# spvkgn/vorbis-aotuv-lancer

Hardware: AMD Instinct MI355X
Metric: realtime-stream-equivalents/node (44.1kHz stereo q5) + MDCT HBM GB/s (higher is better)
Workload: dtype f32

## Files before the change

vorbis_aotuv_lancer_amd/csrc/capi_encoder.cpp:

```cpp
#include <hip/hip_runtime.h>
#include <stdlib.h>
#include <string.h>
#include <functional>
#include <string>
#include <algorithm>
#include <thread>
#include <vector>

#include "vorbis_mi355x.h"
#include "setup_host.h"
#include "batch.h"
#include "kernels.h"
#include "mdct_kernel.h"
#include "vbm_internal.h"

extern "C" int vbm_launch_spread_flags(const vbm_batch *b, hipStream_t st);
vbm_setup_host *vbm_setup_handle_host(vbm_setup_handle *h);

static const int kMaxWS = 8;

struct vbm_encoder {
    vbm_setup_host *H;
    const vbm_setup *hs;
    int S, ch, cap;
// ... 447 lines not shown
    b.mix_makes_qf = vbm_mix_can_make_qf(&b);
    {
        const vbm_map &m = s->map[b.W];
        const vbm_psy &p = s->psy[block_mode];
        unsigned seen = 0;
        b.couple_parallel = 1;
        for (int i = 0; i < m.coupling_steps; i++) {
            unsigned bits = (1u << m.coupling_mag[i]) | (1u << m.coupling_ang[i]);
            if (seen & bits) b.couple_parallel = 0;
            seen |= bits;
        }
        const int partition = p.normal_p ? p.normal_partition : 16;
        int lowpassr = s->block_lowpassr[b.W ? 1 : 0];
        if (lowpassr % p.normal_partition) lowpassr = (lowpassr / p.normal_partition + 1) * p.normal_partition;
        b.couple_parts = (lowpassr + partition - 1) / partition;
        int m6end = p.tonefix_end < lowpassr ? p.tonefix_end : lowpassr;
        b.couple_m6parts = m.coupling_steps ? (m6end + partition - 1) / partition : 0;
        if (b.couple_parts > b.n / 8 + 1) b.couple_parallel = 0;
        b.couple_fast = 0;
        if (partition == 32 && p.normal_partition == 32 && (b.n % 32) == 0) {
            if (m.coupling_steps == 0) b.couple_fast = 1;
            else if (m.coupling_steps == 1 && e->ch == 2 && b.couple_parallel) b.couple_fast = 2;
        }
        b.pack_submaps = m.submaps;
        for (int i = 0; i < m.submaps && i < 16; i++) {
            const vbm_residue &r = s->residue[m.residuesubmap[i]];
            b.pack_partvals[i] = (r.end - r.begin) / r.grouping;
            b.pack_spp[i] = r.grouping;
        }
    }
}

static vbm_batch slice_of(const vbm_batch &f, int sb0, int nsb)
{
    vbm_batch v = f;
    const size_t cb0 = (size_t)sb0 * f.ch;
    const size_t ct = cb0 >> 6, stl = (size_t)sb0 >> 6;
    v.nsb = nsb;
    v.ncb = nsb * f.ch;
    v.stream_id += sb0; v.wflags += sb0;
    v.pcm += cb0 * f.N; v.mdct_bm += cb0 * f.n; v.logfft_bm += cb0 * f.n; v.qf_bm += cb0 * f.n;
    v.local_ampmax += cb0; v.wflags_cb += cb0; v.poste += cb0; v.post_valid += cb0; v.nonzero += cb0;
    v.post_valid_blob += cb0; v.nonzero_blob += cb0;
    v.global_ampmax += sb0; v.packet_bytes += sb0; v.packet_bits += sb0; v.packet_bits_blob += sb0;
    if (v.packet_bytes_blob) { v.packet_bytes_blob += sb0; v.choice += sb0; v.packetT_blob += stl * 64 * (size_t)f.max_packet_bytes; }
    const size_t co = ct * f.slab_words;
    v.mdctT += co; v.logmdctT += co; v.noiseT += co; v.toneT += co; v.logmaskT += co;
    v.epeakT += co; v.npeakT += co;
    v.postT += co; v.postT_blob += co; v.floor_outT += co; v.iworkT += co;
    v.floor_outT_blob += co; v.iworkT_blob += co;
    const size_t so = stl * f.sb_slab_words;
    v.partwordT += so; v.workvqT += so; v.m6defT += so; v.vqlenT += so; v.vqoffT += so;
    v.partwordT_blob += so; v.m6defT_blob += so; v.vqlenT_blob += so; v.vqoffT_blob += so;
    v.vqcodeT += stl * f.vq_slab_words; v.vqcodeT_blob += stl * f.vq_slab_words;
    v.packetT += stl * 64 * (size_t)f.max_packet_bytes;
    return v;
}

static int managed_front(const vbm_batch &v, hipStream_t q)
{
    static const int sel[3] = {1, 2, 0}, slot[3] = {VBM_PACKETBLOBS / 2, VBM_PACKETBLOBS - 1, 0};
    for (int t = 0; t < 3; t++) {
        vbm_batch f = v;
        f.postT = v.postT_blob + (size_t)slot[t] * (VBM_VIF_POSIT + 2) * 64;
        f.post_valid = v.post_valid_blob + (size_t)slot[t] * v.L;
        if (vbm_launch_mix_managed(&f, sel[t], q) || vbm_launch_floor_fit(&f, q)) return -2;
    }
    if (vbm_launch_block_state_managed(&v, q) || vbm_launch_floor_interp(&v, q)) return -2;
    return 0;
}

static int managed_back(const vbm_batch &v, uint8_t *d_packets, hipStream_t q, const std::function<int()> &before_choose = nullptr)
{
    vbm_batch f = v;
    f.nblobs = VBM_PACKETBLOBS;
    vbm_blob_select(f, 0);
    if (vbm_launch_floor_encode(&f, q)) return -2;
    if (f.couple_fast) {
        if (vbm_launch_couple_quantize(&f, q)) return -2;
    } else {
        for (int k = 0; k < VBM_PACKETBLOBS; k++) {
            vbm_batch g = v;
            vbm_blob_select(g, k);
            if (vbm_launch_couple_quantize(&g, q)) return -2;
        }
    }
    if (vbm_launch_pack(&f, q)) return -2;
    if (before_choose && before_choose()) return -2;
    return vbm_launch_bitrate_choose(&v, d_packets, q);
}


static int launch_transforms(vbm_encoder *e, const vbm_batch &v, hipStream_t q, bool timed)
{
    const vbm_setup *d = vbm_setup_device_ptrs(e->H);
    const int W = v.W, short_n = e->hs->blocksizes[0];
    const uint8_t *wf = W ? v.wflags_cb : nullptr;
    RUN(vbm_launch_spread_flags(&v, q));
    {
        stage_scope t(e, timed, 0, q);
        RUN(vbm_launch_window_mdct(v.pcm, v.mdct_bm, wf, d->mdct_trig[W], d->window[W], d->window[0], v.N, short_n, 1, v.ncb,
                                   0, v.d_nsb, e->ch, q));
    }
    stage_scope t(e, timed, 1, q);
    RUN(vbm_launch_window_fft_log(v.pcm, v.logfft_bm, v.local_ampmax, wf, d->fft_wa[W], d->window[W], d->window[0], v.N,
                                  short_n, v.ncb, v.d_nsb, e->ch, q));
    return VBM_OK;
}

static int launch_psy(vbm_encoder *e, const vbm_batch &v, hipStream_t q, bool timed, int side = -1)
{
    const int lines = e->hs->psy[v.block_mode].total_octave_lines;
    hipError_t err;
    { stage_scope t(e, timed, 3, q); RUN(vbm_launch_prologue(&v, q)); }
    if (side >= 0) {
        hipStream_t qa = e->aux[side];
        if ((err = hipEventRecord(e->ev_aux_fork[side], q)) != hipSuccess) return vbm_set_hip_error(err, "hipEventRecord");
        if ((err = hipStreamWaitEvent(qa, e->ev_aux_fork[side], 0)) != hipSuccess) return vbm_set_hip_error(err, "hipStreamWaitEvent");
        { stage_scope t(e, timed, 5, qa); RUN(vbm_launch_tonemask(&v, lines, qa)); }
        if ((err = hipEventRecord(e->ev_aux_join[side], qa)) != hipSuccess) return vbm_set_hip_error(err, "hipEventRecord");
        { stage_scope t(e, timed, 4, q); RUN(vbm_launch_noisemask(&v, q)); }
        if ((err = hipStreamWaitEvent(q, e->ev_aux_join[side], 0)) != hipSuccess) return vbm_set_hip_error(err, "hipStreamWaitEvent");
    } else {
        { stage_scope t(e, timed, 4, q); RUN(vbm_launch_noisemask(&v, q)); }
        { stage_scope t(e, timed, 5, q); RUN(vbm_launch_tonemask(&v, lines, q)); }
    }
    stage_scope t(e, timed, 6, q);
    if (e->hs->managed) RUN(managed_front(v, q));
    else { RUN(vbm_launch_mix(&v, q)); RUN(vbm_launch_block_state(&v, q)); }
    return VBM_OK;
}

static int launch_back(vbm_encoder *e, const vbm_batch &v, hipStream_t q, bool timed, uint8_t *d_packets,
                       const std::function<int()> &before_choose = nullptr)
{
    if (e->hs->managed) {
        stage_scope t(e, timed, 10, q);
        RUN(managed_back(v, d_packets, q, before_choose));
        return VBM_OK;
    }
    { stage_scope t(e, timed, 7, q); RUN(vbm_launch_floor_fit(&v, q)); }
    { stage_scope t(e, timed, 8, q); RUN(vbm_launch_floor_encode(&v, q)); }
    { stage_scope t(e, timed, 9, q); RUN(vbm_launch_couple_quantize(&v, q)); }
    stage_scope t(e, timed, 10, q);
    RUN(vbm_launch_pack(&v, q));
    return VBM_OK;
}

static int copy_packets(vbm_encoder *e, const vbm_batch &v, uint8_t *d_packets, int *d_packet_bytes, int sb0, hipStream_t q,
                        bool timed)
{
    stage_scope t(e, timed, 11, q);
    if (d_packets && !e->hs->managed)
        RUN(vbm_launch_untranspose_i32((const int *)v.packetT, (int *)(d_packets + (size_t)sb0 * e->max_packet_bytes),
                                       e->max_packet_bytes / 4, (size_t)(e->max_packet_bytes / 4) * 64, v.nsb, q));
    if (d_packet_bytes) {
        hipError_t err = hipMemcpyAsync(d_packet_bytes + sb0, v.packet_bytes, v.nsb * sizeof(int), hipMemcpyDeviceToDevice, q);
        if (err != hipSuccess) return vbm_set_hip_error(err, "hipMemcpyAsync(packet_bytes)");
    }
    return VBM_OK;
}

extern "C" int vbm_analysis_batch(vbm_encoder *e, int block_mode, int nsb, const int *stream_ids,
                                  const uint8_t *wflags, const float *d_pcm, uint8_t *d_packets,
                                  int *d_packet_bytes, void *stream)
{
    return vbm_analysis_batch2(e, block_mode, nsb, stream_ids, wflags, d_pcm, d_packets, d_packet_bytes, stream, stream);
}

extern "C" int vbm_analysis_batch2(vbm_encoder *e, int block_mode, int nsb, const int *stream_ids,
                                   const uint8_t *wflags, const float *d_pcm, uint8_t *d_packets,
                                   int *d_packet_bytes, void *stream_front, void *stream_back)
{
    void *stream = stream_front;
    if (!e || block_mode < 0 || block_mode > 3 || nsb < 0 || nsb > e->cap) return VBM_EINVAL;
    if (nsb == 0) return VBM_OK;
    if (!stream_ids || !wflags || !d_pcm) return VBM_EINVAL;
    if (((uintptr_t)d_pcm & 15) || ((uintptr_t)d_packets & 3)) return VBM_EINVAL;
    const vbm_setup *s = e->hs;
    if (s->modes < 2 && (block_mode >> 1)) return VBM_EINVAL;
    for (int i = 0; i < nsb; i++)
        if (stream_ids[i] < 0 || stream_ids[i] >= e->S) return VBM_EINVAL;
    hipStream_t st = (hipStream_t)stream;
    hipStream_t sback = (hipStream_t)stream_back;
    const bool two = (sback != st);
    hipError_t err;
    {
        int rcj = vbm_analysis_round_join(e, stream);
        if (rcj) return rcj;
        for (int ww = 0; ww < e->nws; ww++)
            for (int m = 0; m < 4; m++)
                if (e->reuse_pending[ww][m]) {
                    if ((err = hipStreamWaitEvent((hipStream_t)stream, e->ev_done[ww][m], 0)) != hipSuccess)
                        return vbm_set_hip_error(err, "hipStreamWaitEvent");
                    e->reuse_pending[ww][m] = false;
                }
        e->round_w = -1;
    }
    const int w = e->next;
    e->next = (e->next + 1) % e->nws;
    e->cur = w;
    if (e->back_pending[w]) {
        if ((err = hipStreamWaitEvent(st, e->ev_back[w], 0)) != hipSuccess) return vbm_set_hip_error(err, "hipStreamWaitEvent");
        e->back_pending[w] = false;
    }
    if ((int)e->last_ids[w].size() != nsb || memcmp(e->last_ids[w].data(), stream_ids, nsb * sizeof(int)) ||
        memcmp(e->last_flags[w].data(), wflags, nsb)) {
        e->seen.assign(e->S, 0);
        for (int i = 0; i < nsb; i++) {
            if (e->seen[stream_ids[i]]) { g_vbm_err = "a stream id appears twice in one batch"; return VBM_EINVAL; }
            e->seen[stream_ids[i]] = 1;
        }
        const int t = e->stage_turn;
        e->stage_turn ^= 1;
        (void)hipEventSynchronize(e->ev_stage[t]);
        memcpy(e->h_ids[t], stream_ids, nsb * sizeof(int));
        memcpy(e->h_flags[t], wflags, nsb);
        if ((err = hipMemcpyAsync(e->d_stream_id[w], e->h_ids[t], nsb * sizeof(int), hipMemcpyHostToDevice, st)) != hipSuccess)
            return vbm_set_hip_error(err, "hipMemcpyAsync(stream_ids)");
        if ((err = hipMemcpyAsync(e->d_wflags[w], e->h_flags[t], nsb, hipMemcpyHostToDevice, st)) != hipSuccess)
            return vbm_set_hip_error(err, "hipMemcpyAsync(wflags)");
        (void)hipEventRecord(e->ev_stage[t], st);
        e->last_ids[w].assign(stream_ids, stream_ids + nsb);
        e->last_flags[w].assign(wflags, wflags + nsb);
    }

    vbm_batch b;
    configure(e, b, block_mode, nsb, d_pcm, w);
    e->last_nsb = nsb;
    e->last_mode = block_mode;

    const int tiles = (nsb + 63) / 64;
    int nsplit = e->nsplit < tiles ? e->nsplit : tiles;
    if (nsplit < 1) nsplit = 1;
    const int nback = nsplit;
    if (two) nsplit = 1;

    int rc;
    const size_t ev_need = (size_t)2 * (kFront + (size_t)(nsplit > nback ? nsplit : nback) * kBack);
    const bool prof = e->profiling && e->prof_calls < e->prof_max_calls && e->events_used + ev_need <= e->events.size();
    vbm_debug_delay_point(VBM_DP_BATCH_FRONT, st);
    if ((rc = launch_transforms(e, b, st, prof))) return rc;
    if (two) {
        if ((rc = launch_psy(e, b, st, prof, e->overlap_branches ? 0 : -1))) return rc;
        if ((err = hipEventRecord(e->ev_front[w], st)) != hipSuccess) return vbm_set_hip_error(err, "hipEventRecord");
        for (int part = 0; part < nback; part++) {
            const int t0 = (int)((long)tiles * part / nback), t1 = (int)((long)tiles * (part + 1) / nback);
            const int sb0 = t0 * 64, sb1 = (t1 * 64 < nsb) ? t1 * 64 : nsb;
            if (sb1 <= sb0) continue;
            hipStream_t qb = part ? e->sub[part] : sback;
            if ((err = hipStreamWaitEvent(qb, e->ev_front[w], 0)) != hipSuccess) return vbm_set_hip_error(err, "hipStreamWaitEvent");
            vbm_debug_delay_point(VBM_DP_BATCH_BACK, qb);
            vbm_batch vs = nback > 1 ? slice_of(b, sb0, sb1 - sb0) : b;
            if ((rc = launch_back(e, vs, qb, prof, d_packets ? d_packets + (size_t)sb0 * e->max_packet_bytes : nullptr)) ||
                (rc = copy_packets(e, vs, d_packets, d_packet_bytes, sb0, qb, prof)))
                return rc;
            if (part) {
                if ((err = hipEventRecord(e->ev_join[part], qb)) != hipSuccess) return vbm_set_hip_error(err, "hipEventRecord");
                if ((err = hipStreamWaitEvent(sback, e->ev_join[part], 0)) != hipSuccess) return vbm_set_hip_error(err, "hipStreamWaitEvent");
            }
        }
        if ((err = hipEventRecord(e->ev_back[w], sback)) != hipSuccess) return vbm_set_hip_error(err, "hipEventRecord");
        e->back_pending[w] = true;
    } else {
        if (nsplit > 1 && (err = hipEventRecord(e->ev_fork, st)) != hipSuccess) return vbm_set_hip_error(err, "hipEventRecord");
        for (int part = 0; part < nsplit; part++) {
            const int t0 = (int)((long)tiles * part / nsplit), t1 = (int)((long)tiles * (part + 1) / nsplit);
            const int sb0 = t0 * 64, sb1 = (t1 * 64 < nsb) ? t1 * 64 : nsb;
            if (sb1 <= sb0) continue;
            hipStream_t q = st;
            vbm_batch v = b;
            if (nsplit > 1) {
                q = e->sub[part];
                v = slice_of(b, sb0, sb1 - sb0);
                if ((err = hipStreamWaitEvent(q, e->ev_fork, 0)) != hipSuccess) return vbm_set_hip_error(err, "hipStreamWaitEvent");
            }
            if ((rc = launch_psy(e, v, q, prof, e->overlap_branches ? part : -1)) ||
                (rc = launch_back(e, v, q, prof, d_packets ? d_packets + (size_t)sb0 * e->max_packet_bytes : nullptr)) ||
                (rc = copy_packets(e, v, d_packets, d_packet_bytes, sb0, q, prof)))
                return rc;
            if (nsplit > 1) {
                if ((err = hipEventRecord(e->ev_join[part], q)) != hipSuccess) return vbm_set_hip_error(err, "hipEventRecord");
                if ((err = hipStreamWaitEvent(st, e->ev_join[part], 0)) != hipSuccess) return vbm_set_hip_error(err, "hipStreamWaitEvent");
            }
        }
    }
    if (prof) { e->prof_calls++; e->prof_blocks += nsb; }
    return VBM_OK;
}

struct type_job {
    int m, w;
    int lane0, bound;
    const int *d_nsb;
    const float *pcm;
    uint8_t *d_packets;
    int *d_packet_bytes;
    bool big, timed;
    unsigned depmask;
    int few = 0;
    int part = 0;
    bool grouped = false;
    hipStream_t q_on = nullptr;
};

static vbm_batch job_batch(vbm_encoder *e, const type_job &j)
{
    vbm_batch full;
// ... 630 lines not shown
```

vorbis_aotuv_lancer_amd/csrc/kernels.h:

```cpp
#pragma once
#include <hip/hip_runtime.h>
#include "batch.h"

extern "C" {
int vbm_launch_transpose_in(const vbm_batch *b, hipStream_t st);
int vbm_launch_prologue(const vbm_batch *b, hipStream_t st);
int vbm_launch_noisemask(const vbm_batch *b, hipStream_t st);
int vbm_launch_tonemask(const vbm_batch *b, int total_octave_lines, hipStream_t st);
int vbm_launch_mix(const vbm_batch *b, hipStream_t st);
int vbm_mix_can_make_qf(const vbm_batch *b);
int vbm_launch_reset_streams(const vbm_stream_state *st, const int *d_ids, int n, long long bm_fill, hipStream_t q);
int vbm_launch_block_state(const vbm_batch *b, hipStream_t st);
int vbm_launch_mix_managed(const vbm_batch *b, int offset_select, hipStream_t st);
int vbm_launch_block_state_managed(const vbm_batch *b, hipStream_t st);
int vbm_launch_floor_interp(const vbm_batch *b, hipStream_t st);
int vbm_launch_bitrate_choose(const vbm_batch *b, uint8_t *d_packets, hipStream_t st);
int vbm_launch_floor_fit(const vbm_batch *b, hipStream_t st);
int vbm_launch_floor_encode(const vbm_batch *b, hipStream_t st);
int vbm_launch_couple_quantize(const vbm_batch *b, hipStream_t st);
int vbm_launch_pack(const vbm_batch *b, hipStream_t st);
int vbm_launch_packets_out(const vbm_batch *b, uint8_t *dst, int *dst_bytes, hipStream_t st);
int vbm_launch_pack_head(const vbm_batch *b, hipStream_t st);
int vbm_launch_pack_residue(const vbm_batch *b, hipStream_t st);
int vbm_launch_untranspose_f32(const float *srcT, float *dst_bm, int rows, size_t slab, int ncols, hipStream_t st);
int vbm_launch_untranspose_i32(const int *srcT, int *dst_bm, int rows, size_t slab, int ncols, hipStream_t st);
int vbm_launch_compact(const uint8_t *rows, const int *len, int n, int maxb, long long *off, uint8_t *out, hipStream_t q);
int vbm_launch_untranspose_counted(const int *srcT, int *dst_bm, int rows, size_t slab, int ncols, const int *d_ncols, hipStream_t st);
int vbm_launch_copy_counted(int *dst, const int *src, int n, const int *d_count, hipStream_t st);
int vbm_launch_untranspose_u8(const uint8_t *srcT, uint8_t *dst_bm, int rows, size_t slab, int ncols, hipStream_t st);
}
```

vorbis_aotuv_lancer_amd/csrc/pack_kernels.hip:

```cpp
#include <hip/hip_runtime.h>
#include <stdint.h>
#include "batch.h"
#include "kernels.h"

namespace {

struct BitW {
    uint32_t *base;
    int nwords, maxwords;
    uint64_t acc;
    int nbits;
};

__device__ __forceinline__ void bw_write(BitW &w, uint32_t value, int bits)
{
    if (bits <= 0) return;
    if (bits < 32) value &= (1u << bits) - 1u;
    w.acc |= (uint64_t)value << w.nbits;
    w.nbits += bits;
    if (w.nbits >= 32) {
        if (w.nwords < w.maxwords) w.base[(size_t)w.nwords * 64] = (uint32_t)w.acc;
        w.acc >>= 32;
        w.nbits -= 32;
        w.nwords++;
    }
}

__device__ __forceinline__ int bw_finish(BitW &w)
{
    if (w.nbits > 0 && w.nwords < w.maxwords) w.base[(size_t)w.nwords * 64] = (uint32_t)w.acc;
    return w.nwords * 32 + w.nbits;
}

__device__ __forceinline__ void or_bits(uint32_t *words, int maxwords, int pos, uint32_t value, int bits)
{
    if (bits <= 0) return;
    if (bits < 32) value &= (1u << bits) - 1u;
    const uint64_t v = (uint64_t)value << (pos & 31);
    const int wi = pos >> 5;
    if (wi < maxwords) atomicOr(&words[(size_t)wi * 64], (uint32_t)v);
    if ((v >> 32) && wi + 1 < maxwords) atomicOr(&words[(size_t)(wi + 1) * 64], (uint32_t)(v >> 32));
}

__device__ __forceinline__ int ilog(uint32_t v)
{
    return v ? 32 - __clz(v) : 0;
}

__device__ __forceinline__ int book_encode(const vbm_book *bk, int a, BitW &w)
{
    if (a < 0 || a >= bk->entries) return 0;
    bw_write(w, bk->codelist[a], bk->lengthlist[a]);
    return bk->lengthlist[a];
}

struct book_regs {
    int dim, minval, delta, quantvals, used, entries;
    const signed char *lengthlist;
    const uint32_t *codelist;
    const int *used_point, *used_index;
    const short *used_pack;
    const int *used_norm;
};
__device__ __forceinline__ book_regs load_book(const vbm_book *book)
{
    book_regs r;
    r.dim = book->dim; r.minval = book->minval; r.delta = book->delta; r.quantvals = book->quantvals;
    r.used = book->used; r.entries = book->entries;
    r.lengthlist = book->lengthlist; r.codelist = book->codelist;
    r.used_point = book->used_point; r.used_index = book->used_index;
    r.used_pack = book->used_pack; r.used_norm = book->used_norm;
    return r;
}

__device__ __forceinline__ int div_trunc(int num, int den)
{
    if (abs(num) < (1 << 23)) return (int)((float)num / (float)den);
    return num / den;
}

__device__ __forceinline__ int besterror(const book_regs *book, int *a)
{
    const int dim = book->dim;
    int i, j, o;
    const int minval = book->minval, del = book->delta, qv = book->quantvals;
    const int ze = (qv >> 1);
    int index = 0;
    int p[VBM_MAX_BOOK_DIM] = {0, 0, 0, 0, 0, 0, 0, 0};

    if (del != 1) {
        for (i = 0, o = dim; i < dim; i++) {
            int v = div_trunc(a[--o] - minval + (del >> 1), del);
            int m = (v < ze ? ((ze - v) << 1) - 1 : ((v - ze) << 1));
            index = index * qv + (m < 0 ? 0 : (m >= qv ? qv - 1 : m));
            p[o] = v * del + minval;
        }
    } else {
        for (i = 0, o = dim; i < dim; i++) {
            int v = a[--o] - minval;
            int m = (v < ze ? ((ze - v) << 1) - 1 : ((v - ze) << 1));
            index = index * qv + (m < 0 ? 0 : (m >= qv ? qv - 1 : m));
            p[o] = v * del + minval;
        }
    }

    if (book->lengthlist[index] <= 0) {
        const int used = book->used;
        int bi = 0;
        bool small = book->used_pack != nullptr;
        for (j = 0; j < dim; j++) small = small && (a[j] >= -32768 && a[j] <= 32767);
        if (small) {
            typedef short short2v __attribute__((ext_vector_type(2)));
            uint32_t pa[4] = {0u, 0u, 0u, 0u};
            for (j = 0; j < dim; j++) pa[j >> 1] |= ((uint32_t)a[j] & 0xffffu) << ((j & 1) * 16);
            const uint4 *pk = reinterpret_cast<const uint4 *>(book->used_pack);
            const int *__restrict__ nrm = book->used_norm;
            const int words = (dim + 1) >> 1;
            int best = 0;
            for (i = 0; i < used; i++) {
                const uint4 v = pk[i];
                int dot = __builtin_amdgcn_sdot2(__builtin_bit_cast(short2v, v.x), __builtin_bit_cast(short2v, pa[0]), 0, false);
                if (words > 1) dot = __builtin_amdgcn_sdot2(__builtin_bit_cast(short2v, v.y), __builtin_bit_cast(short2v, pa[1]), dot, false);
                if (words > 2) {
                    dot = __builtin_amdgcn_sdot2(__builtin_bit_cast(short2v, v.z), __builtin_bit_cast(short2v, pa[2]), dot, false);
                    dot = __builtin_amdgcn_sdot2(__builtin_bit_cast(short2v, v.w), __builtin_bit_cast(short2v, pa[3]), dot, false);
                }
                const int score = nrm[i] - 2 * dot;
                if (i == 0 || score < best) { best = score; bi = i; }
            }
        } else {
            int best = -1;
            const int *pt = book->used_point;
            for (i = 0; i < used; i++, pt += dim) {
                int dist = 0;
                for (j = 0; j < dim; j++) {
                    int val = pt[j] - a[j];
                    dist += val * val;
                }
                if (best == -1 || dist < best) { best = dist; bi = i; }
            }
        }
        if (used > 0) {
            const int *pt = book->used_point + (size_t)bi * dim;
            for (j = 0; j < dim; j++) p[j] = pt[j];
            index = book->used_index[bi];
        }
    }

    if (index > -1)
        for (i = 0; i < dim; i++) a[i] -= p[i];
    return index;
}

struct res_view {
    const vbm_residue *r;
    int nb;
    int chlist[VBM_MAXCH];
    int used;
    int vch[VBM_MAXCH];
    int partvals, spp;
};

__device__ __forceinline__ res_view residue_view(const vbm_batch &b, const vbm_map *info, int sm, size_t col0)
{
    res_view v;
    v.r = &b.setup->residue[info->residuesubmap[sm]];
    v.nb = 0;
    v.used = 0;
    int any = 0;
    for (int j = 0; j < b.ch; j++)
        if (info->chmuxlist[j] == sm) {
            const int nz = b.nonzero[col0 + j] ? 1 : 0;
            v.chlist[v.nb++] = j;
            any |= nz;
            if (nz && v.r->type != 2) v.vch[v.used++] = j;
        }
    if (v.r->type == 2) v.used = any ? 1 : 0;
    v.spp = v.r->grouping;
    v.partvals = (v.r->end - v.r->begin) / v.spp;
    return v;
}

#define SBT(sb) ((size_t)((sb) >> 6) * b.sb_slab_words + ((sb) & 63))
#define IWC(cc, x) b.iworkT[(size_t)((col0 + (cc)) >> 6) * b.slab_words + (size_t)(x) * 64 + ((col0 + (cc)) & 63)]
#define PW(jv, iv) partword[((size_t)(jv) * v.partvals + (iv)) * 64]
#define LEN(stg, jv, iv) lenT[(((size_t)(stg) * b.ch + (jv)) * v.partvals + (iv)) * 64]
#define OFF(stg, jv, iv) offT[(((size_t)(stg) * b.ch + (jv)) * v.partvals + (iv)) * 64]

template <bool BLOBS>
__global__ void k_nonzero_propagate(vbm_batch b)
{
    vbm_blob_enter<BLOBS>(b);
    const int sb = blockIdx.x * blockDim.x + threadIdx.x;
    if (sb >= vbm_nsb(b)) return;
// ... 264 lines not shown
        const bool live = c < vbm_nsb(b);
        const int k = live ? b.choice[c] : 0;
        const int len = live ? b.packet_bytes[c] : 0;
        const uint32_t *src = (const uint32_t *)(b.packetT_blob + (size_t)k * blob_stride) + (size_t)(c >> 6) * rows * 64 + (c & 63);
        for (int rr = ty; rr < 64; rr += 4) {
            const int r = r0 + rr;
            uint32_t w = 0;
            if (live && r < rows && r * 4 < len) {
                w = src[(size_t)r * 64];
                const int keep = len - r * 4;
                if (keep < 4) w &= (1u << (8 * keep)) - 1u;
            }
            tile[rr][tx] = w;
        }
    }
    __syncthreads();
    for (int cc = ty; cc < 64; cc += 4) {
        const int c = c0 + cc, r = r0 + tx;
        if (c < vbm_nsb(b) && r < rows) dst[(size_t)c * rows + r] = tile[tx][cc];
    }
}

__device__ __forceinline__ void res_classify(const vbm_batch &b, const res_view &v, const int sb, const size_t col0, const int i0, const int i1)
{
    const vbm_residue *r = v.r;
    int *partword = b.partwordT + SBT(sb);
    const int possible_partitions = r->partitions;
    const int rbegin = r->begin;
    const int *__restrict__ classmetric1 = r->classmetric1, *__restrict__ classmetric2 = r->classmetric2;
    int i, j, k;

    if (r->type == 2) {
        const int nb = v.nb;
        const int lsteps = (v.spp + nb - 1) / nb;
        for (i = i0; i < i1; i++) {
            int magmax = 0, angmax = 0;
            int l = rbegin / nb + i * lsteps;
            for (j = 0; j < v.spp; j += nb, l++) {
                int v0 = abs(IWC(v.chlist[0], l));
                if (v0 > magmax) magmax = v0;
                for (k = 1; k < nb; k++) {
                    int vk = abs(IWC(v.chlist[k], l));
                    if (vk > angmax) angmax = vk;
                }
            }
            for (j = 0; j < possible_partitions - 1; j++)
                if (magmax <= classmetric1[j] && angmax <= classmetric2[j]) break;
            PW(0, i) = j;
        }
    } else {
        const float scale = (float)(100. / v.spp);
        for (i = i0; i < i1; i++) {
            const int offset = i * v.spp + rbegin;
            for (j = 0; j < v.used; j++) {
                int mx = 0, ent = 0;
                for (k = 0; k < v.spp; k++) {
                    int a = abs(IWC(v.vch[j], offset + k));
                    if (a > mx) mx = a;
                    ent += a;
                }
                ent = (int)((float)ent * scale);
                for (k = 0; k < possible_partitions - 1; k++)
                    if (mx <= classmetric1[k] && (classmetric2[k] < 0 || ent < classmetric2[k])) break;
                PW(j, i) = k;
            }
        }
    }
}

template <bool BLOBS>
__global__ void k_res_vq(vbm_batch b, int sm, int nchunks)
{
    vbm_blob_enter<BLOBS>(b);
    extern __shared__ int vq_lds[];
    const int sb = blockIdx.x * blockDim.x + threadIdx.x;
    if (sb >= vbm_nsb(b)) return;
    const vbm_setup *s = b.setup;
    const vbm_map *info = &s->map[b.W];
    const size_t col0 = (size_t)sb * b.ch;
    const res_view v = residue_view(b, info, sm, col0);
    if (!v.used) return;
    const vbm_residue *r = v.r;
    const int i0 = (int)((long)v.partvals * blockIdx.y / nchunks), i1 = (int)((long)v.partvals * (blockIdx.y + 1) / nchunks);
    res_classify(b, v, sb, col0, i0, i1);
    const int *partword = b.partwordT + SBT(sb);
    int *lenT = b.vqlenT + SBT(sb);
    uint64_t *slot = b.vqcodeT + (size_t)(sb >> 6) * b.vq_slab_words + (sb & 63);
    const int veclen = (r->type == 2) ? b.n * v.nb : b.n;
    const size_t stage_slots = (size_t)b.n * b.ch;
    int *stage = vq_lds + threadIdx.x;
    const int spp = v.spp, nb = v.nb, rbegin = r->begin;

    for (int i = i0; i < i1; i++) {
        const int offset = i * spp + rbegin;
        for (int j = 0; j < v.used; j++) {
            if (r->type == 2) {
                int l = offset / nb, k = offset - l * nb;
                for (int e = 0; e < spp; e++) {
                    stage[e * 64] = IWC(v.chlist[k], l);
                    if (++k == nb) { k = 0; l++; }
                }
            } else {
                for (int e = 0; e < spp; e++) stage[e * 64] = IWC(v.vch[j], offset + e);
            }
            const int cls = PW(j, i);
            for (int st = 0; st < r->stages; st++) {
                int bits = 0;
                const int bi = (r->secondstages[cls] & (1 << st)) ? r->partbook[cls][st] : -1;
                if (bi >= 0) {
                    const book_regs bk = load_book(&s->book[bi]);
                    const book_regs *book = &bk;
                    const int dim = book->dim;
                    const int step = spp / dim;
                    uint64_t *sl = slot + (st * stage_slots + (size_t)j * veclen + offset) * 64;
                    for (int t = 0; t < step; t++) {
                        int a[VBM_MAX_BOOK_DIM];
                        int *src = stage + t * dim * 64;
                        for (int d = 0; d < dim; d++) a[d] = src[d * 64];
                        const int entry = besterror(book, a);
                        for (int d = 0; d < dim; d++) src[d * 64] = a[d];
                        uint64_t cw = 0;
                        if (entry >= 0 && entry < book->entries) {
                            const int len = book->lengthlist[entry];
                            cw = (uint64_t)book->codelist[entry] | ((uint64_t)(uint32_t)len << 32);
                            bits += len;
                        }
                        sl[(size_t)t * 64] = cw;
                    }
                }
                LEN(st, j, i) = bits;
            }
        }
    }
}

template <bool BLOBS>
__global__ void k_res_offsets(vbm_batch b, int sm)
{
    vbm_blob_enter<BLOBS>(b);
    const int sb = blockIdx.x * blockDim.x + threadIdx.x;
    if (sb >= vbm_nsb(b)) return;
    const vbm_setup *s = b.setup;
    const vbm_map *info = &s->map[b.W];
    const size_t col0 = (size_t)sb * b.ch;
    const res_view v = residue_view(b, info, sm, col0);
    const int maxwords = b.max_packet_bytes / 4;
    int pos = b.packet_bits[sb];
    if (v.used) {
        const vbm_residue *r = v.r;
        const int *partword = b.partwordT + SBT(sb);
        const int *lenT = b.vqlenT + SBT(sb);
        int *offT = b.vqoffT + SBT(sb);
        uint32_t *words = (uint32_t *)b.packetT + (size_t)(sb >> 6) * maxwords * 64 + (sb & 63);
        const vbm_book *phrasebook = &s->book[r->groupbook];
        const int partitions_per_word = r->phrase_dim;
        if (v.used == 1 && partitions_per_word == 2) {
            const signed char *__restrict__ pll = phrasebook->lengthlist;
            const uint32_t *__restrict__ pcl = phrasebook->codelist;
            const int pents = phrasebook->entries, nparts = r->partitions, pv = v.partvals;
            for (int st = 0; st < r->stages; st++) {
                for (int i = 0; i < pv; i += 16) {
                    int plen[8], l0[8], l1[8];
                    uint32_t pcode[8];
#pragma unroll
                    for (int g = 0; g < 8; g++) {
                        const int ia = i + 2 * g, ib = ia + 1;
                        plen[g] = 0; pcode[g] = 0;
                        if (st == 0 && ia < pv) {
                            long val = (long)PW(0, ia) * nparts;
                            if (ib < pv) val += PW(0, ib);
                            if (val < pents) { plen[g] = pll[val]; pcode[g] = pcl[val]; }
                        }
                        l0[g] = (ia < pv) ? LEN(st, 0, ia) : 0;
                        l1[g] = (ib < pv) ? LEN(st, 0, ib) : 0;
                    }
#pragma unroll
                    for (int g = 0; g < 8; g++) {
                        const int ia = i + 2 * g, ib = ia + 1;
                        if (ia < pv) {
                            if (st == 0 && plen[g] > 0) {
                                or_bits(words, maxwords, pos, pcode[g], plen[g]);
                                pos += plen[g];
                            }
                            OFF(st, 0, ia) = pos;
                            pos += l0[g];
                            if (ib < pv) {
                                OFF(st, 0, ib) = pos;
                                pos += l1[g];
                            }
                        }
                    }
                }
            }
        } else
        for (int st = 0; st < r->stages; st++) {
            for (int i = 0; i < v.partvals;) {
                if (st == 0) {
                    for (int j = 0; j < v.used; j++) {
                        long val = PW(j, i);
                        for (int k = 1; k < partitions_per_word; k++) {
                            val *= r->partitions;
                            if (i + k < v.partvals) val += PW(j, i + k);
                        }
                        if (val < phrasebook->entries) {
                            const int len = phrasebook->lengthlist[val];
                            or_bits(words, maxwords, pos, phrasebook->codelist[val], len);
                            pos += len;
                        }
                    }
                }
                for (int k = 0; k < partitions_per_word && i < v.partvals; k++, i++)
                    for (int j = 0; j < v.used; j++) {
                        OFF(st, j, i) = pos;
                        pos += LEN(st, j, i);
                    }
            }
        }
        b.packet_bits[sb] = pos;
    }
    b.packet_bytes[sb] = (pos > maxwords * 32) ? -1 : (pos + 7) / 8;
}

template <bool BLOBS>
__global__ void k_res_emit(vbm_batch b, int sm, int nchunks)
{
    vbm_blob_enter<BLOBS>(b);
    const int sb = blockIdx.x * blockDim.x + threadIdx.x;
    if (sb >= vbm_nsb(b)) return;
    const vbm_map *info = &b.setup->map[b.W];
    const size_t col0 = (size_t)sb * b.ch;
    const res_view v = residue_view(b, info, sm, col0);
    if (!v.used) return;
    const vbm_residue *r = v.r;
    const int i0 = (int)((long)v.partvals * blockIdx.y / nchunks), i1 = (int)((long)v.partvals * (blockIdx.y + 1) / nchunks);
    const int *lenT = b.vqlenT + SBT(sb);
    const int *offT = b.vqoffT + SBT(sb);
    const uint64_t *slot = b.vqcodeT + (size_t)(sb >> 6) * b.vq_slab_words + (sb & 63);
    const int maxwords = b.max_packet_bytes / 4;
    uint32_t *words = (uint32_t *)b.packetT + (size_t)(sb >> 6) * maxwords * 64 + (sb & 63);
    const int veclen = (r->type == 2) ? b.n * v.nb : b.n;
    const size_t stage_slots = (size_t)b.n * b.ch;

    for (int st = 0; st < r->stages; st++)
        for (int i = i0; i < i1; i++) {
            const int offset = i * v.spp + r->begin;
            for (int j = 0; j < v.used; j++) {
                int remaining = LEN(st, j, i);
                if (remaining <= 0) continue;
                const int pos = OFF(st, j, i);
                const uint64_t *sl = slot + (st * stage_slots + (size_t)j * veclen + offset) * 64;
                int wi = pos >> 5;
                int nbits = pos & 31;
                uint64_t acc = 0;
                for (int t0 = 0; t0 < v.spp && remaining > 0; t0 += 8) {
                    uint64_t cwv[8];
#pragma unroll
                    for (int u = 0; u < 8; u++) cwv[u] = sl[(size_t)((t0 + u < v.spp) ? t0 + u : v.spp - 1) * 64];
#pragma unroll
                    for (int u = 0; u < 8; u++) {
                        if (t0 + u < v.spp && remaining > 0) {
                            const uint64_t cw = cwv[u];
                            const int len = (int)(cw >> 32);
                            if (len) {
                                acc |= (uint64_t)(uint32_t)cw << nbits;
                                nbits += len;
                                remaining -= len;
                                if (nbits >= 32) {
                                    if (wi < maxwords) atomicOr(&words[(size_t)wi * 64], (uint32_t)acc);
                                    acc >>= 32;
                                    nbits -= 32;
                                    wi++;
                                }
                            }
                        }
                    }
                }
                if (nbits > 0 && wi < maxwords) atomicOr(&words[(size_t)wi * 64], (uint32_t)acc);
            }
        }
}


}

extern "C" int vbm_launch_block_state(const vbm_batch *b, hipStream_t st)
{
    hipLaunchKernelGGL(k_block_state, dim3((unsigned)((b->nsb + 63) / 64)), dim3(64), 0, st, *b, 1);
    return hipGetLastError() == hipSuccess ? 0 : -2;
}
extern "C" int vbm_launch_block_state_managed(const vbm_batch *b, hipStream_t st)
{
    hipLaunchKernelGGL(k_block_state, dim3((unsigned)((b->nsb + 63) / 64)), dim3(64), 0, st, *b, VBM_PACKETBLOBS);
    return hipGetLastError() == hipSuccess ? 0 : -2;
}
extern "C" int vbm_launch_bitrate_choose(const vbm_batch *b, uint8_t *d_packets, hipStream_t st)
{
    hipLaunchKernelGGL(k_bitrate_choose, dim3((unsigned)((b->nsb + 63) / 64)), dim3(64), 0, st, *b);
    if (d_packets) {
        const int rows = b->max_packet_bytes / 4;
        hipLaunchKernelGGL(k_blob_gather, dim3((unsigned)((b->nsb + 63) / 64), (unsigned)((rows + 63) / 64)), dim3(256), 0, st,
                           *b, (uint32_t *)d_packets);
    }
    return hipGetLastError() == hipSuccess ? 0 : -2;
}

static __global__ void k_zero_u128(uint4 *__restrict__ p, size_t n, size_t blob_stride)
{
    const size_t i = (size_t)blockIdx.x * blockDim.x + threadIdx.x;
    if (i < n) p[(size_t)blockIdx.z * blob_stride + i] = make_uint4(0u, 0u, 0u, 0u);
}

extern "C" int vbm_launch_pack_head(const vbm_batch *b, hipStream_t st)
{
    const unsigned tiles = (unsigned)((b->nsb + 63) / 64);
    const unsigned nbl = (unsigned)(b->nblobs > 1 ? b->nblobs : 1);
    {
        const size_t n16 = (size_t)tiles * 64 * b->max_packet_bytes / 16;
        hipLaunchKernelGGL(k_zero_u128, dim3((unsigned)((n16 + 255) / 256), 1, nbl), dim3(256), 0, st, (uint4 *)b->packetT, n16,
                           (size_t)b->Ls * b->max_packet_bytes / 16);
    }
    if (nbl > 1) hipLaunchKernelGGL(k_pack_head<true>, dim3(tiles, 1, nbl), dim3(64), 0, st, *b);
    else hipLaunchKernelGGL(k_pack_head<false>, dim3(tiles), dim3(64), 0, st, *b);
    return hipGetLastError() == hipSuccess ? 0 : -2;
}

extern "C" int vbm_launch_pack_residue(const vbm_batch *b, hipStream_t st)
{
    const unsigned tiles = (unsigned)((b->nsb + 63) / 64);
    const unsigned nbl = (unsigned)(b->nblobs > 1 ? b->nblobs : 1);
    if (nbl > 1) hipLaunchKernelGGL(k_nonzero_propagate<true>, dim3(tiles, 1, nbl), dim3(64), 0, st, *b);
    else hipLaunchKernelGGL(k_nonzero_propagate<false>, dim3(tiles), dim3(64), 0, st, *b);
    for (int sm = 0; sm < b->pack_submaps; sm++) {
        const int most = (b->few || b->nsb <= 1024) ? 256 : 32;
        int nchunks = b->pack_partvals[sm] < most ? b->pack_partvals[sm] : most;
        if (nchunks < 1) nchunks = 1;
        const size_t lds = (size_t)b->pack_spp[sm] * 64 * sizeof(int);
        if (nbl > 1) {
            hipLaunchKernelGGL(k_res_vq<true>, dim3(tiles, (unsigned)nchunks, nbl), dim3(64), lds, st, *b, sm, nchunks);
            hipLaunchKernelGGL(k_res_offsets<true>, dim3(tiles, 1, nbl), dim3(64), 0, st, *b, sm);
            hipLaunchKernelGGL(k_res_emit<true>, dim3(tiles, (unsigned)nchunks, nbl), dim3(64), 0, st, *b, sm, nchunks);
        } else {
            hipLaunchKernelGGL(k_res_vq<false>, dim3(tiles, (unsigned)nchunks), dim3(64), lds, st, *b, sm, nchunks);
            hipLaunchKernelGGL(k_res_offsets<false>, dim3(tiles), dim3(64), 0, st, *b, sm);
            hipLaunchKernelGGL(k_res_emit<false>, dim3(tiles, (unsigned)nchunks), dim3(64), 0, st, *b, sm, nchunks);
        }
    }
    return hipGetLastError() == hipSuccess ? 0 : -2;
}

extern "C" int vbm_launch_pack(const vbm_batch *b, hipStream_t st)
{
    int rc = vbm_launch_pack_head(b, st);
    return rc ? rc : vbm_launch_pack_residue(b, st);
}

extern "C" int vbm_launch_packets_out(const vbm_batch *b, uint8_t *dst, int *dst_bytes, hipStream_t st)
{
    int rc = 0;
    if (dst) rc = vbm_launch_untranspose_counted((const int *)b->packetT, (int *)dst, b->max_packet_bytes / 4,
                                                 (size_t)(b->max_packet_bytes / 4) * 64, b->nsb, b->d_nsb, st);
    if (!rc && dst_bytes) rc = vbm_launch_copy_counted(dst_bytes, b->packet_bytes, b->nsb, b->d_nsb, st);
    return rc;
}
```

vorbis_aotuv_lancer_amd/csrc/util_kernels.hip:

```cpp
#include <hip/hip_runtime.h>
#include <stdint.h>
#include "batch.h"
#include "kernels.h"

namespace {

template <typename T>
__global__ void k_to_tiled(const T *__restrict__ src, T *__restrict__ dst, int ncols, int rows, size_t slab)
{
    __shared__ T tile[64][65];
    const int c0 = blockIdx.x * 64, r0 = blockIdx.y * 64;
    const int tx = threadIdx.x & 63, ty = threadIdx.x >> 6;
    for (int cc = ty; cc < 64; cc += 4) {
        int c = c0 + cc, r = r0 + tx;
        tile[cc][tx] = (c < ncols && r < rows) ? src[(size_t)c * rows + r] : T(0);
    }
    __syncthreads();
    for (int rr = ty; rr < 64; rr += 4) {
        int r = r0 + rr, c = c0 + tx;
        if (r < rows && c < ncols) dst[(size_t)(c >> 6) * slab + (size_t)r * 64 + (c & 63)] = tile[tx][rr];
    }
}

template <typename T>
__global__ void k_from_tiled(const T *__restrict__ src, T *__restrict__ dst, int ncols, int rows, size_t slab,
                             const int *__restrict__ d_ncols)
{
    if (d_ncols) ncols = *d_ncols;
    if ((int)(blockIdx.x * 64) >= ncols) return;
    __shared__ T tile[64][65];
    const int c0 = blockIdx.x * 64, r0 = blockIdx.y * 64;
    const int tx = threadIdx.x & 63, ty = threadIdx.x >> 6;
    for (int rr = ty; rr < 64; rr += 4) {
        int r = r0 + rr, c = c0 + tx;
        tile[rr][tx] = (r < rows && c < ncols) ? src[(size_t)(c >> 6) * slab + (size_t)r * 64 + (c & 63)] : T(0);
    }
    __syncthreads();
    for (int cc = ty; cc < 64; cc += 4) {
        int c = c0 + cc, r = r0 + tx;
        if (c < ncols && r < rows) dst[(size_t)c * rows + r] = tile[tx][cc];
    }
}

__global__ void k_copy_counted(int *__restrict__ dst, const int *__restrict__ src, int n, const int *__restrict__ d_count)
{
    if (d_count) n = *d_count;
    const int i = blockIdx.x * blockDim.x + threadIdx.x;
    if (i < n) dst[i] = src[i];
}

__global__ void k_spread_flags(const uint8_t *__restrict__ wflags, uint8_t *__restrict__ wflags_cb, int nsb, int ch)
{
    int i = blockIdx.x * blockDim.x + threadIdx.x;
    if (i < nsb * ch) wflags_cb[i] = wflags[i / ch];
}

template <typename T>
int to_tiled(const T *src, T *dst, int ncols, int rows, size_t slab, hipStream_t st)
{
    dim3 grid((unsigned)((ncols + 63) / 64), (unsigned)((rows + 63) / 64));
    hipLaunchKernelGGL(k_to_tiled<T>, grid, dim3(256), 0, st, src, dst, ncols, rows, slab);
    return hipGetLastError() == hipSuccess ? 0 : -2;
}

template <typename T>
int from_tiled(const T *src, T *dst, int ncols, int rows, size_t slab, hipStream_t st, const int *d_ncols = nullptr)
{
    dim3 grid((unsigned)((ncols + 63) / 64), (unsigned)((rows + 63) / 64));
    hipLaunchKernelGGL(k_from_tiled<T>, grid, dim3(256), 0, st, src, dst, ncols, rows, slab, d_ncols);
    return hipGetLastError() == hipSuccess ? 0 : -2;
}

__global__ void k_reset_streams(vbm_stream_state st, const int *__restrict__ ids, int n, long long bm_fill)
{
    const int lane = blockIdx.x * blockDim.x + threadIdx.x;
    if (lane >= n * st.ch) return;
    const int s = ids[lane / st.ch], ci = lane % st.ch;
    const int col = s * st.ch + ci;
    float *mb = st.mblock + (size_t)(col >> 6) * st.slab_words + (col & 63);
    for (int i = 0; i < 2048 + 256; i++) mb[(size_t)i * 64] = 0.f;
    st.lowcomp[col] = 0.f;
    if (ci == 0) {
        st.g_ampmax[s] = -9999.f;
        st.vbi_ampmax[s] = -9999.f;
        st.lW_block_mode[s] = 0;
        st.lW_no[s] = 0;
        st.impadnum[s] = 0;
        st.bm_avg_reservoir[s] = bm_fill;
        st.bm_minmax_reservoir[s] = bm_fill;
        st.bm_avgfloat[s] = (double)(VBM_PACKETBLOBS / 2);
    }
}

__global__ __launch_bounds__(1024) void k_compact_scan(const int *__restrict__ len, int n, long long *__restrict__ off)
{
    __shared__ long long s_part[16];
    __shared__ long long s_carry;
    const int lane = threadIdx.x & 63, wave = threadIdx.x >> 6;
    if (threadIdx.x == 0) s_carry = 0;
    __syncthreads();
    for (int base = 0; base < n; base += 1024) {
        const int k = base + threadIdx.x;
        int l = k < n ? len[k] : 0;
        if (l < 0) l = 0;
        long long v = (l + 3) & ~3, incl = v;
#pragma unroll
        for (int d = 1; d < 64; d <<= 1) {
            long long t = __shfl_up(incl, d);
            if (lane >= d) incl += t;
        }
        if (lane == 63) s_part[wave] = incl;
        __syncthreads();
        long long before = s_carry;
        for (int w = 0; w < wave; w++) before += s_part[w];
        if (k < n) off[k] = before + incl - v;
        __syncthreads();
        if (threadIdx.x == 1023) s_carry = before + incl;
        __syncthreads();
    }
    if (threadIdx.x == 0) off[n] = s_carry;
}

__global__ void k_compact_copy(const uint8_t *__restrict__ rows, const int *__restrict__ len, int n, int maxb,
                               const long long *__restrict__ off, uint8_t *__restrict__ out)
{
    const int k = blockIdx.x * (blockDim.x >> 6) + (threadIdx.x >> 6), lane = threadIdx.x & 63;
    if (k >= n) return;
    const int l = len[k];
    if (l <= 0) return;
    const uint32_t *src = (const uint32_t *)(rows + (size_t)k * maxb);
    uint32_t *dst = (uint32_t *)(out + off[k]);
    for (int w = lane; w < (l + 3) / 4; w += 64) dst[w] = src[w];
}

}

extern "C" int vbm_launch_compact(const uint8_t *rows, const int *len, int n, int maxb, long long *off, uint8_t *out,
                                  hipStream_t q)
{
    if (n <= 0) return 0;
    hipLaunchKernelGGL(k_compact_scan, dim3(1), dim3(1024), 0, q, len, n, off);
    hipLaunchKernelGGL(k_compact_copy, dim3((unsigned)((n + 3) / 4)), dim3(256), 0, q, rows, len, n, maxb, off, out);
    return hipGetLastError() == hipSuccess ? 0 : -2;
}

extern "C" int vbm_launch_reset_streams(const vbm_stream_state *st, const int *d_ids, int n, long long bm_fill, hipStream_t q)
{
    if (n <= 0) return 0;
    hipLaunchKernelGGL(k_reset_streams, dim3((unsigned)((n * st->ch + 63) / 64)), dim3(64), 0, q, *st, d_ids, n, bm_fill);
    return hipGetLastError() == hipSuccess ? 0 : -2;
}

extern "C" int vbm_launch_spread_flags(const vbm_batch *b, hipStream_t st)
{
    hipLaunchKernelGGL(k_spread_flags, dim3((unsigned)((b->ncb + 255) / 256)), dim3(256), 0, st, b->wflags,
                       b->wflags_cb, b->nsb, b->ch);
    return hipGetLastError() == hipSuccess ? 0 : -2;
}

extern "C" int vbm_launch_transpose_in(const vbm_batch *b, hipStream_t st)
{
    return to_tiled<float>(b->mdct_bm, b->mdctT, b->ncb, b->n, b->slab_words, st);
}

extern "C" int vbm_launch_untranspose_f32(const float *srcT, float *dst_bm, int rows, size_t slab, int ncols,
                                          hipStream_t st)
{
    return from_tiled<float>(srcT, dst_bm, ncols, rows, slab, st);
}
extern "C" int vbm_launch_untranspose_i32(const int *srcT, int *dst_bm, int rows, size_t slab, int ncols,
                                          hipStream_t st)
{
    return from_tiled<int>(srcT, dst_bm, ncols, rows, slab, st);
}
extern "C" int vbm_launch_untranspose_counted(const int *srcT, int *dst_bm, int rows, size_t slab, int ncols,
                                              const int *d_ncols, hipStream_t st)
{
    return from_tiled<int>(srcT, dst_bm, ncols, rows, slab, st, d_ncols);
}
extern "C" int vbm_launch_copy_counted(int *dst, const int *src, int n, const int *d_count, hipStream_t st)
{
    if (n <= 0) return 0;
    hipLaunchKernelGGL(k_copy_counted, dim3((unsigned)((n + 255) / 256)), dim3(256), 0, st, dst, src, n, d_count);
    return hipGetLastError() == hipSuccess ? 0 : -2;
}
extern "C" int vbm_launch_untranspose_u8(const uint8_t *srcT, uint8_t *dst_bm, int rows, size_t slab, int ncols,
                                         hipStream_t st)
{
    return from_tiled<uint8_t>(srcT, dst_bm, ncols, rows, slab, st);
}

namespace {
__global__ void k_stamp(unsigned long long *out, int slot, int tag)
{
    out[2 * slot] = (unsigned long long)tag;
    out[2 * slot + 1] = wall_clock64();
}
unsigned long long *g_stamps = nullptr;
int g_stamp_next = 0, g_stamp_on = -1;
const int kStampMax = 8192;
}
extern "C" void vbm_debug_stamp(hipStream_t st, int tag)
{
    if (g_stamp_on < 0) g_stamp_on = getenv("VBM_DEBUG_STAMPS") ? 1 : 0;
    if (!g_stamp_on) return;
    if (!g_stamps && hipMalloc((void **)&g_stamps, (size_t)kStampMax * 16) != hipSuccess) { g_stamp_on = 0; return; }
    if (g_stamp_next >= kStampMax) return;
    hipLaunchKernelGGL(k_stamp, dim3(1), dim3(1), 0, st, g_stamps, g_stamp_next++, tag);
}
extern "C" int vbm_debug_stamps_read(unsigned long long *out, int max_pairs)
{
    if (!g_stamps) return 0;
    (void)hipDeviceSynchronize();
    const int n = g_stamp_next < max_pairs ? g_stamp_next : max_pairs;
    (void)hipMemcpy(out, g_stamps, (size_t)n * 16, hipMemcpyDeviceToHost);
    return n;
}
```

Measured before the change: 84110.

## Skip packet buffer pre-zeroing; clear words lazily and copy only used packet words

The separate zero-fill kernel over the whole tiled packet buffer now runs only in the multi-blob path. In the single-blob path the residue offset kernel clears words as it advances its write position. The untranspose of packets is replaced by a kernel that reads only the words each packet actually uses, based on packet_bytes, and writes zeros for the rest. This cuts HBM traffic from the full-buffer memset and from reading unused packet words. The cost is extra per-word stores inside the bit writer and a reliance on every writer path clearing its words correctly.

```diff
diff --git a/vorbis_aotuv_lancer_amd/csrc/capi_encoder.cpp b/vorbis_aotuv_lancer_amd/csrc/capi_encoder.cpp
--- a/vorbis_aotuv_lancer_amd/csrc/capi_encoder.cpp
+++ b/vorbis_aotuv_lancer_amd/csrc/capi_encoder.cpp
@@ -623,8 +623,8 @@
 {
     stage_scope t(e, timed, 11, q);
     if (d_packets && !e->hs->managed)
-        RUN(vbm_launch_untranspose_i32((const int *)v.packetT, (int *)(d_packets + (size_t)sb0 * e->max_packet_bytes),
-                                       e->max_packet_bytes / 4, (size_t)(e->max_packet_bytes / 4) * 64, v.nsb, q));
+        RUN(vbm_launch_packet_rows((const int *)v.packetT, v.packet_bytes, (int *)(d_packets + (size_t)sb0 * e->max_packet_bytes),
+                                   e->max_packet_bytes / 4, v.nsb, nullptr, q));
     if (d_packet_bytes) {
         hipError_t err = hipMemcpyAsync(d_packet_bytes + sb0, v.packet_bytes, v.nsb * sizeof(int), hipMemcpyDeviceToDevice, q);
         if (err != hipSuccess) return vbm_set_hip_error(err, "hipMemcpyAsync(packet_bytes)");
diff --git a/vorbis_aotuv_lancer_amd/csrc/kernels.h b/vorbis_aotuv_lancer_amd/csrc/kernels.h
--- a/vorbis_aotuv_lancer_amd/csrc/kernels.h
+++ b/vorbis_aotuv_lancer_amd/csrc/kernels.h
@@ -25,7 +25,7 @@
 int vbm_launch_untranspose_f32(const float *srcT, float *dst_bm, int rows, size_t slab, int ncols, hipStream_t st);
 int vbm_launch_untranspose_i32(const int *srcT, int *dst_bm, int rows, size_t slab, int ncols, hipStream_t st);
 int vbm_launch_compact(const uint8_t *rows, const int *len, int n, int maxb, long long *off, uint8_t *out, hipStream_t q);
-int vbm_launch_untranspose_counted(const int *srcT, int *dst_bm, int rows, size_t slab, int ncols, const int *d_ncols, hipStream_t st);
+int vbm_launch_packet_rows(const int *packetT, const int *packet_bytes, int *dst, int rows, int ncols, const int *d_ncols, hipStream_t st);
 int vbm_launch_copy_counted(int *dst, const int *src, int n, const int *d_count, hipStream_t st);
 int vbm_launch_untranspose_u8(const uint8_t *srcT, uint8_t *dst_bm, int rows, size_t slab, int ncols, hipStream_t st);
 }
diff --git a/vorbis_aotuv_lancer_amd/csrc/pack_kernels.hip b/vorbis_aotuv_lancer_amd/csrc/pack_kernels.hip
--- a/vorbis_aotuv_lancer_amd/csrc/pack_kernels.hip
+++ b/vorbis_aotuv_lancer_amd/csrc/pack_kernels.hip
@@ -40,6 +40,22 @@
     const int wi = pos >> 5;
     if (wi < maxwords) atomicOr(&words[(size_t)wi * 64], (uint32_t)v);
     if ((v >> 32) && wi + 1 < maxwords) atomicOr(&words[(size_t)(wi + 1) * 64], (uint32_t)(v >> 32));
+}
+
+template <bool CLEAR>
+__device__ __forceinline__ void fresh_to(uint32_t *words, int maxwords, int &zw, int endbit)
+{
+    if (!CLEAR) return;
+    int e = (endbit + 31) >> 5;
+    if (e > maxwords) e = maxwords;
+    for (; zw < e; zw++) words[(size_t)zw * 64] = 0u;
+}
+template <bool CLEAR>
+__device__ __forceinline__ void or_bits_fresh(uint32_t *words, int maxwords, int &zw, int pos, uint32_t value, int bits)
+{
+    if (bits <= 0) return;
+    fresh_to<CLEAR>(words, maxwords, zw, pos + bits);
+    or_bits(words, maxwords, pos, value, bits);
 }
 
 __device__ __forceinline__ int ilog(uint32_t v)
@@ -610,6 +626,7 @@
         const int *lenT = b.vqlenT + SBT(sb);
         int *offT = b.vqoffT + SBT(sb);
         uint32_t *words = (uint32_t *)b.packetT + (size_t)(sb >> 6) * maxwords * 64 + (sb & 63);
+        int zw = (pos + 31) >> 5;
         const vbm_book *phrasebook = &s->book[r->groupbook];
         const int partitions_per_word = r->phrase_dim;
         if (v.used == 1 && partitions_per_word == 2) {
@@ -637,7 +654,7 @@
                         const int ia = i + 2 * g, ib = ia + 1;
                         if (ia < pv) {
                             if (st == 0 && plen[g] > 0) {
-                                or_bits(words, maxwords, pos, pcode[g], plen[g]);
+                                or_bits_fresh<!BLOBS>(words, maxwords, zw, pos, pcode[g], plen[g]);
                                 pos += plen[g];
                             }
                             OFF(st, 0, ia) = pos;
@@ -662,7 +679,7 @@
                         }
                         if (val < phrasebook->entries) {
                             const int len = phrasebook->lengthlist[val];
-                            or_bits(words, maxwords, pos, phrasebook->codelist[val], len);
+                            or_bits_fresh<!BLOBS>(words, maxwords, zw, pos, phrasebook->codelist[val], len);
                             pos += len;
                         }
                     }
@@ -674,6 +691,7 @@
                     }
             }
         }
+        fresh_to<!BLOBS>(words, maxwords, zw, pos);
         b.packet_bits[sb] = pos;
     }
     b.packet_bytes[sb] = (pos > maxwords * 32) ? -1 : (pos + 7) / 8;
@@ -762,23 +780,24 @@
     return hipGetLastError() == hipSuccess ? 0 : -2;
 }
 
-static __global__ void k_zero_u128(uint4 *__restrict__ p, size_t n, size_t blob_stride)
+static __global__ void k_zero_u128(uint4 *__restrict__ p, size_t n, size_t tile16, size_t blob_stride, const int *__restrict__ d_nsb)
 {
     const size_t i = (size_t)blockIdx.x * blockDim.x + threadIdx.x;
-    if (i < n) p[(size_t)blockIdx.z * blob_stride + i] = make_uint4(0u, 0u, 0u, 0u);
+    if (i >= n || (d_nsb && i / tile16 >= (size_t)((*d_nsb + 63) / 64))) return;
+    p[(size_t)blockIdx.z * blob_stride + i] = make_uint4(0u, 0u, 0u, 0u);
 }
 
 extern "C" int vbm_launch_pack_head(const vbm_batch *b, hipStream_t st)
 {
     const unsigned tiles = (unsigned)((b->nsb + 63) / 64);
     const unsigned nbl = (unsigned)(b->nblobs > 1 ? b->nblobs : 1);
-    {
-        const size_t n16 = (size_t)tiles * 64 * b->max_packet_bytes / 16;
+    if (nbl > 1) {
+        const size_t tile16 = (size_t)64 * b->max_packet_bytes / 16;
+        const size_t n16 = (size_t)tiles * tile16;
         hipLaunchKernelGGL(k_zero_u128, dim3((unsigned)((n16 + 255) / 256), 1, nbl), dim3(256), 0, st, (uint4 *)b->packetT, n16,
-                           (size_t)b->Ls * b->max_packet_bytes / 16);
-    }
-    if (nbl > 1) hipLaunchKernelGGL(k_pack_head<true>, dim3(tiles, 1, nbl), dim3(64), 0, st, *b);
-    else hipLaunchKernelGGL(k_pack_head<false>, dim3(tiles), dim3(64), 0, st, *b);
+                           tile16, (size_t)b->Ls * b->max_packet_bytes / 16, b->d_nsb);
+        hipLaunchKernelGGL(k_pack_head<true>, dim3(tiles, 1, nbl), dim3(64), 0, st, *b);
+    } else hipLaunchKernelGGL(k_pack_head<false>, dim3(tiles), dim3(64), 0, st, *b);
     return hipGetLastError() == hipSuccess ? 0 : -2;
 }
 
@@ -815,8 +834,8 @@
 extern "C" int vbm_launch_packets_out(const vbm_batch *b, uint8_t *dst, int *dst_bytes, hipStream_t st)
 {
     int rc = 0;
-    if (dst) rc = vbm_launch_untranspose_counted((const int *)b->packetT, (int *)dst, b->max_packet_bytes / 4,
-                                                 (size_t)(b->max_packet_bytes / 4) * 64, b->nsb, b->d_nsb, st);
+    if (dst) rc = vbm_launch_packet_rows((const int *)b->packetT, b->packet_bytes, (int *)dst, b->max_packet_bytes / 4, b->nsb,
+                                         b->d_nsb, st);
     if (!rc && dst_bytes) rc = vbm_launch_copy_counted(dst_bytes, b->packet_bytes, b->nsb, b->d_nsb, st);
     return rc;
 }
diff --git a/vorbis_aotuv_lancer_amd/csrc/util_kernels.hip b/vorbis_aotuv_lancer_amd/csrc/util_kernels.hip
--- a/vorbis_aotuv_lancer_amd/csrc/util_kernels.hip
+++ b/vorbis_aotuv_lancer_amd/csrc/util_kernels.hip
@@ -23,11 +23,8 @@
 }
 
 template <typename T>
-__global__ void k_from_tiled(const T *__restrict__ src, T *__restrict__ dst, int ncols, int rows, size_t slab,
-                             const int *__restrict__ d_ncols)
-{
-    if (d_ncols) ncols = *d_ncols;
-    if ((int)(blockIdx.x * 64) >= ncols) return;
+__global__ void k_from_tiled(const T *__restrict__ src, T *__restrict__ dst, int ncols, int rows, size_t slab)
+{
     __shared__ T tile[64][65];
     const int c0 = blockIdx.x * 64, r0 = blockIdx.y * 64;
     const int tx = threadIdx.x & 63, ty = threadIdx.x >> 6;
@@ -42,6 +39,35 @@
     }
 }
 
+__global__ void k_packet_rows(const int *__restrict__ src, const int *__restrict__ len, int *__restrict__ dst, int ncols,
+                              int rows, const int *__restrict__ d_ncols)
+{
+    if (d_ncols) ncols = *d_ncols;
+    if ((int)(blockIdx.x * 64) >= ncols) return;
+    __shared__ int tile[64][65];
+    const int c0 = blockIdx.x * 64, r0 = blockIdx.y * 64;
+    const int tx = threadIdx.x & 63, ty = threadIdx.x >> 6;
+    {
+        const int c = c0 + tx;
+        int words = 0;
+        if (c < ncols) {
+            const int l = len[c];
+            words = l < 0 ? rows : (l + 3) >> 2;
+            if (words > rows) words = rows;
+        }
+        const int *col = src + (size_t)(c >> 6) * rows * 64 + (c & 63);
+        for (int rr = ty; rr < 64; rr += 4) {
+            const int r = r0 + rr;
+            tile[rr][tx] = r < words ? col[(size_t)r * 64] : 0;
+        }
+    }
+    __syncthreads();
+    for (int cc = ty; cc < 64; cc += 4) {
+        int c = c0 + cc, r = r0 + tx;
+        if (c < ncols && r < rows) dst[(size_t)c * rows + r] = tile[tx][cc];
+    }
+}
+
 __global__ void k_copy_counted(int *__restrict__ dst, const int *__restrict__ src, int n, const int *__restrict__ d_count)
 {
     if (d_count) n = *d_count;
@@ -64,10 +90,10 @@
 }
 
 template <typename T>
-int from_tiled(const T *src, T *dst, int ncols, int rows, size_t slab, hipStream_t st, const int *d_ncols = nullptr)
+int from_tiled(const T *src, T *dst, int ncols, int rows, size_t slab, hipStream_t st)
 {
     dim3 grid((unsigned)((ncols + 63) / 64), (unsigned)((rows + 63) / 64));
-    hipLaunchKernelGGL(k_from_tiled<T>, grid, dim3(256), 0, st, src, dst, ncols, rows, slab, d_ncols);
+    hipLaunchKernelGGL(k_from_tiled<T>, grid, dim3(256), 0, st, src, dst, ncols, rows, slab);
     return hipGetLastError() == hipSuccess ? 0 : -2;
 }
 
@@ -173,10 +199,13 @@
 {
     return from_tiled<int>(srcT, dst_bm, ncols, rows, slab, st);
 }
-extern "C" int vbm_launch_untranspose_counted(const int *srcT, int *dst_bm, int rows, size_t slab, int ncols,
-                                              const int *d_ncols, hipStream_t st)
-{
-    return from_tiled<int>(srcT, dst_bm, ncols, rows, slab, st, d_ncols);
+extern "C" int vbm_launch_packet_rows(const int *packetT, const int *packet_bytes, int *dst, int rows, int ncols,
+                                      const int *d_ncols, hipStream_t st)
+{
+    if (ncols <= 0) return 0;
+    dim3 grid((unsigned)((ncols + 63) / 64), (unsigned)((rows + 63) / 64));
+    hipLaunchKernelGGL(k_packet_rows, grid, dim3(256), 0, st, packetT, packet_bytes, dst, ncols, rows, d_ncols);
+    return hipGetLastError() == hipSuccess ? 0 : -2;
 }
 extern "C" int vbm_launch_copy_counted(int *dst, const int *src, int n, const int *d_count, hipStream_t st)
 {
```

Measured after the change: 88820 (median of 6 runs). 1.06x the previous value.
